# Disty0/sdnq

Hardware: AMD Instinct MI355X
Metric: quantized-matmul GOP/s (SDXL UNet int8 Linear step, bs=1) (higher is better)
Workload: dtype i8; 1 GPU; sdxl_int8: 741 quantized Linear layers of one denoising step, bs=1 (722 w8a8 GEMMs + 19 M=1 layers); parallelism=single GPU, launch=hipGraph replay, activations=bf16, distinct_activation_tensors=446, activation_quant_cache=True, requantized_weight_cache=True, fused_projections=False, linked_projection_groups=71, one_launch_linears=232, weights_dtype=int8, group_size=-1, use_quantized_matmul=True

## Files before the change

include/sdnq_hip.h:

```cpp
#ifndef SDNQ_HIP_H
#define SDNQ_HIP_H

#include <stddef.h>
#include <stdint.h>

#ifdef __cplusplus
extern "C" {
#endif

#define SDNQ_HIP_ABI_VERSION 1

typedef void* sdnq_stream_t;

typedef enum SdnqStatus {
    SDNQ_OK = 0,
    SDNQ_ERR_NULL = -1,
    SDNQ_ERR_DTYPE = -2,
    SDNQ_ERR_SHAPE = -3,
    SDNQ_ERR_ALIGN = -4,
    SDNQ_ERR_UNSUPPORTED = -5,
    SDNQ_ERR_ARCH = -6,
    SDNQ_ERR_LAUNCH = -7,
    SDNQ_ERR_WORKSPACE = -8
} SdnqStatus;
// ... 135 lines not shown
int sdnq_hip_lowrank_down(const void* x, int x_dtype, int64_t m, int64_t k, int64_t ldx, const void* svd_down,
                          int svd_dtype, int rank, void* t, sdnq_stream_t stream);

int sdnq_hip_scaled_mm_lowrank(int mm_dtype, const void* a, const void* b, const float* sa, const float* sb,
                               const void* bias, int bias_dtype, const void* t, const void* svd_up, int svd_dtype,
                               int rank, const int32_t* zp_rowsum, const float* zp, const float* a_zp,
                               const float* w_colsum_scaled, void* out, int out_dtype,
                               int64_t m, int64_t n, int64_t k, sdnq_stream_t stream);

int sdnq_hip_linear_float(const void* x, const void* wd, const void* bias, int dtype, void* out, int64_t m,
                          int64_t n, int64_t k, int64_t ldx, sdnq_stream_t stream);

int sdnq_hip_linear_skinny(const SdnqWeight* w, int hadamard_group, const void* x, const void* bias, int dtype, void* out,
                           int64_t m, int64_t ldx, sdnq_stream_t stream);

int sdnq_hip_quantize_weight(const void* src, int src_dtype, int64_t ld_src, const SdnqWeight* w, float qmin,
                             float qmax, sdnq_stream_t stream);

int sdnq_hip_quantize_codebook(const void* src, int src_dtype, int64_t ld_src, const SdnqWeight* w, int steps, sdnq_stream_t stream);

int sdnq_hip_prefetch(const void* ptr, int64_t bytes, int workgroups, sdnq_stream_t stream);
int sdnq_hip_prefetch_hint(const void* p0, int64_t b0, const void* p1, int64_t b1, const void* p2, int64_t b2, const void* p3, int64_t b3);

#define SDNQ_MAX_TP_RANKS 64
int sdnq_hip_unshard_columns(const void* gathered, void* out, int elem_bytes, int64_t m0, int64_t m_rows, int64_t m,
                             int64_t wmax, int world, const int64_t* starts, sdnq_stream_t stream);

#define SDNQ_MAX_PUSH_RANKS 16
#define SDNQ_SIGNAL_UNCACHED 1
#define SDNQ_SIGNAL_FINEGRAINED 2
#define SDNQ_SIGNAL_HOST_COHERENT 3
int sdnq_hip_signal_alloc(int64_t bytes, int kind, void** ptr, int* granted);
int sdnq_hip_signal_free(void* ptr, int kind);
int sdnq_hip_ipc_export(const void* ptr, void* handle64);
int sdnq_hip_ipc_import(const void* handle64, void** ptr);
int sdnq_hip_ipc_close(void* ptr);
int sdnq_hip_push_post(void* const* post, int world, int rank, uint64_t seq, uint64_t arena_offset, sdnq_stream_t stream);
int sdnq_hip_push_columns(const void* y, int elem_bytes, int64_t rows, int64_t w, int64_t ldy, void* const* arena, void* const* post,
                          void* const* done, int world, int rank, uint64_t seq, int64_t ldc, int64_t col0, int64_t row0, void* ticket,
                          void* status, int timeout_ms, sdnq_stream_t stream);

int sdnq_hip_im2col(const void* x, int dtype, int batch, int channels, int height, int width, int kh, int kw, int stride_h,
                    int stride_w, int pad_h, int pad_w, int dil_h, int dil_w, void* out, sdnq_stream_t stream);

int sdnq_hip_linear_w8a8(int mm_dtype, const void* x, int x_dtype, int64_t m, int64_t k, int64_t ldx, int hadamard_group,
                         void* xq, float* xs, const void* b, const float* sb, const void* bias, int bias_dtype, void* out,
                         int out_dtype, int64_t n, sdnq_stream_t stream);

int sdnq_hip_stream_capture_id(sdnq_stream_t stream, unsigned long long* id);

int sdnq_hip_linear_w8a8_fused(int mm_dtype, const void* x, int x_dtype, int64_t m, int64_t k, int64_t ldx, const void* b, const float* sb,
                               const void* bias, int bias_dtype, void* out, int out_dtype, int64_t n, sdnq_stream_t stream);
int sdnq_hip_linear_w8a8_fused_supported(int mm_dtype, int x_dtype, int out_dtype, int64_t m, int64_t n, int64_t k);

typedef struct SdnqLinearArgs {
    int32_t struct_size;
    int32_t mm_dtype;
    int32_t x_dtype;
    int32_t out_dtype;
    int32_t bias_dtype;
    int32_t svd_dtype;
    int32_t hadamard_group;
    int32_t svd_rank;
    int32_t asymmetric;
    int32_t x_prequantized;
    int64_t m, n, k, ldx;
    const void* x;
    void* out;
    const void* wq;
    const float* ws;
    const void* bias;
    const void* svd_down;
    const void* svd_up;
    const float* zp;
    const float* w_colsum_scaled;
    void* xq;
    float* xs;
    int32_t* rowsum;
    void* xrot;
    float* xzp;
    void* workspace;
    int64_t workspace_bytes;
} SdnqLinearArgs;
int sdnq_hip_linear(const SdnqLinearArgs* args, sdnq_stream_t stream);
int sdnq_hip_linear_workspace_bytes(const SdnqLinearArgs* args, int64_t* bytes);

int sdnq_hip_scaled_mm_nchw(int mm_dtype, const void* a, const void* b, const float* sa, const float* sb, const void* bias,
                            int bias_dtype, void* out, int out_dtype, int64_t m, int64_t n, int64_t k, int64_t hw,
                            sdnq_stream_t stream);

int sdnq_hip_scaled_mm_strided(int mm_dtype, const void* a, int64_t lda, const void* b, const float* sa, const float* sb,
                               const void* bias, int bias_dtype, void* out, int64_t ldc, int out_dtype, int64_t m, int64_t n,
                               int64_t k, int64_t hw, sdnq_stream_t stream);

int sdnq_hip_scaled_mm_lowrank_strided(int mm_dtype, const void* a, int64_t lda, const void* b, const float* sa, const float* sb,
                                       const void* bias, int bias_dtype, const int32_t* zp_rowsum, const float* zp, const float* a_zp,
                                       const float* w_colsum_scaled, int64_t zp_k, void* out, int64_t ldc, int out_dtype, int64_t m,
                                       int64_t n, int64_t k, sdnq_stream_t stream);

int sdnq_hip_linear_float_strided(const void* x, const void* wd, const void* bias, int dtype, void* out, int64_t m,
                                  int64_t n, int64_t k, int64_t ldx, int64_t ldc, sdnq_stream_t stream);

int sdnq_hip_im2col_rowquant(const void* x, int dtype, int batch, int channels, int height, int width, int kh, int kw,
                             int stride_h, int stride_w, int pad_h, int pad_w, int dil_h, int dil_w, int mm_dtype,
                             void* xq, float* xs, void* amax_ws, sdnq_stream_t stream);

// ... 127 lines not shown
```

sdnq_amd/csrc/gemm_aq.hip:

```cpp
#include "gemm_dev.h"
#include "quant8_dev.h"

namespace {

constexpr int BK = 128, NW = 8, NT = NW * 64;

struct AqParams {
    const float* sb;
    const void* bias;
    void* out;
    int64_t ldc;
    int bias_dtype;
    const uint8_t* pf_ptr[4];
    int pf_lines[4];
    unsigned long long* trace;
#ifdef SDNQ_AQ_LAB
    int lab;
#endif
};

typedef unsigned short us2 __attribute__((ext_vector_type(2)));

template <int MM> struct AqMma;
template <> struct AqMma<SDNQ_MM_I8> {
// ... 332 lines not shown
std::atomic<int> g_aq_geometry{-1};

constexpr int64_t AQ_TALL_MAX_K = 640;

struct AqPlan { int geometry, bm, bn, tiles_m, tiles_n, group_m, resident; int64_t prefetch_room; };
inline AqPlan aq_plan(int mm_dtype, int64_t m, int64_t n, int64_t k, int cus) {
    static const int geo_env = (int)env_int("SDNQ_HIP_FUSED_ROWQUANT_GEOMETRY", -1);
    static const int gm_env = (int)env_int("SDNQ_HIP_FUSED_ROWQUANT_GROUP_M", 8);
    static const int gm_tall_env = (int)env_int("SDNQ_HIP_FUSED_ROWQUANT_GROUP_M_TALL", 8);
    static const int tall = env_int("SDNQ_HIP_FUSED_ROWQUANT_TALL_GEOMETRY", 2) == 3 ? 3 : 2;
    struct Geo { int bm, bn, resident; };
    static constexpr Geo GEOS[4] = {{64, 128, 1}, {32, 256, 1}, {64, 128, 2}, {128, 128, 1}};
    const bool tall_ok = mm_dtype == SDNQ_MM_I8 && k <= AQ_TALL_MAX_K;
    auto tiles_of = [&](int g) { return ((m + GEOS[g].bm - 1) / GEOS[g].bm) * ((n + GEOS[g].bn - 1) / GEOS[g].bn); };
    int geo = g_aq_geometry.load(std::memory_order_relaxed);
    if (geo < 0) geo = geo_env;
    if (geo > 3 || (geo >= 2 && !tall_ok)) geo = -1;
    if (geo < 0) {
        if (mm_dtype == SDNQ_MM_I8 && k > 640 && (n % 256) == 0 && ((m + 31) / 32) * (n / 256) <= cus) geo = 1;
        else if (tall_ok && tiles_of(0) > cus && tiles_of(tall) <= (int64_t)GEOS[tall].resident * cus) geo = tall;
        else geo = 0;
    }
    AqPlan pl;
    pl.geometry = geo;
    pl.bm = GEOS[geo].bm;
    pl.bn = GEOS[geo].bn;
    pl.resident = GEOS[geo].resident;
    pl.tiles_m = (int)((m + pl.bm - 1) / pl.bm);
    pl.tiles_n = (int)((n + pl.bn - 1) / pl.bn);
    const int gm_e = geo >= 2 ? gm_tall_env : gm_env;
    const int gm = gm_e < 1 ? 1 : gm_e;
    pl.group_m = gm > pl.tiles_m ? pl.tiles_m : gm;
    pl.prefetch_room = (int64_t)pl.resident * cus - (int64_t)pl.tiles_m * pl.tiles_n;
    return pl;
}

template <int X_T, int MM, bool HAS_BIAS, int NJ, int NSB, int BM, int BN, int RESIDENT = 1>
int launch_aq(const void* x, const void* w, int64_t ldx, int64_t m, int64_t n, int64_t k, const AqPlan& pl, AqParams p, hipStream_t s) {
    constexpr int LDS_BYTES = NJ * BM * BK + NSB * BN * BK + (2 * BN + BM) * 4;
    static_assert(RESIDENT * LDS_BYTES <= 160 * 1024 && (RESIDENT + 1) * LDS_BYTES > 160 * 1024, "LDS budget: exactly RESIDENT workgroups per CU (aq_plan's prefetch room)");
    auto kern = linear_aq_kernel<X_T, MM, HAS_BIAS, NJ, NSB, BM, BN>;
    static std::atomic<uint64_t> attr_devices{0};
    if (LDS_BYTES > 64 * 1024 && !allow_dynamic_lds((const void*)kern, LDS_BYTES, attr_devices)) return SDNQ_ERR_LAUNCH;
    if (pl.bm != BM || pl.bn != BN || pl.resident != RESIDENT) return SDNQ_ERR_LAUNCH;
    const int tiles_m = pl.tiles_m, tiles_n = pl.tiles_n, group_m = pl.group_m;
    const int64_t tiles = (int64_t)tiles_m * tiles_n;
    p.trace = g_aq_trace.load(std::memory_order_relaxed);
#ifdef SDNQ_AQ_LAB
    p.lab = (int)env_int("SDNQ_HIP_AQ_LAB", 0);
#endif
    const int pf_wgs = sdnq_internal_take_prefetch(pl.prefetch_room, NT, p.pf_ptr, p.pf_lines);
    hipLaunchKernelGGL(kern, dim3((unsigned)(tiles + pf_wgs)), dim3(NT), LDS_BYTES, s, (const uint16_t*)x, (const uint8_t*)w, (int)ldx, (int)k, (int)m,
                       (int)n, (int)k, tiles_m, tiles_n, group_m, p);
    SDNQ_CHECK_LAUNCH();
    return SDNQ_OK;
}

}

extern "C" int sdnq_hip_linear_w8a8_fused_supported(int mm_dtype, int x_dtype, int out_dtype, int64_t m, int64_t n, int64_t k) {
    static const int64_t on = env_int("SDNQ_HIP_FUSED_ROWQUANT", 1), max_tn = env_int("SDNQ_HIP_FUSED_ROWQUANT_MAX_TILES_N", 12),
                         min_m = env_int("SDNQ_HIP_FUSED_ROWQUANT_MIN_M", 33), min_k = env_int("SDNQ_HIP_FUSED_ROWQUANT_MIN_K", 128),
                         max_k = env_int("SDNQ_HIP_FUSED_ROWQUANT_MAX_K", 1280);
    static const int64_t fp8_on = env_int("SDNQ_HIP_FUSED_ROWQUANT_FP8", 0);
    if (!on) return 0;
    if (mm_dtype != SDNQ_MM_I8 && !(mm_dtype == SDNQ_MM_FP8 && fp8_on)) return 0;
    if ((x_dtype != SDNQ_BF16 && x_dtype != SDNQ_F16) || out_dtype != x_dtype) return 0;
    if (m < min_m || n <= 0 || (n % 8) != 0 || k <= 0 || (k % 128) != 0 || k > 1280) return 0;
    const int64_t tiles_m = (m + 63) / 64, tiles_n = (n + 127) / 128;
    if (tiles_n > max_tn || k < min_k || k > max_k) return 0;
    if (tiles_m * tiles_n > (int64_t)cu_count() && aq_plan(mm_dtype, m, n, k, cu_count()).geometry < 2) return 0;
    return 1;
}

extern "C" int sdnq_hip_linear_w8a8_fused(int mm_dtype, const void* x, int x_dtype, int64_t m, int64_t k, int64_t ldx, const void* b,
                                          const float* sb, const void* bias, int bias_dtype, void* out, int out_dtype, int64_t n,
                                          sdnq_stream_t stream) {
    if (!x || !b || !sb || !out) return SDNQ_ERR_NULL;
    if (mm_dtype != SDNQ_MM_I8 && mm_dtype != SDNQ_MM_FP8) return SDNQ_ERR_DTYPE;
    if ((x_dtype != SDNQ_BF16 && x_dtype != SDNQ_F16) || out_dtype != x_dtype) return SDNQ_ERR_UNSUPPORTED;
    if (bias && (bias_dtype < 0 || bias_dtype > 2)) return SDNQ_ERR_DTYPE;
    if (m <= 0 || n <= 0 || k <= 0 || ldx < k || (n % 8) != 0) return SDNQ_ERR_SHAPE;
    if ((k % 128) != 0 || k > 1280) return SDNQ_ERR_UNSUPPORTED;
    if (m > 0x7fffffffll / 2 || n > 0x7fffffffll || ldx * 2 * 128 > 0x7fffffffll || k * 128 > 0x7fffffffll) return SDNQ_ERR_SHAPE;
    if (((uintptr_t)x % 16) || ((uintptr_t)b % 16) || ((uintptr_t)out % 16) || ((ldx * 2) % 16)) return SDNQ_ERR_ALIGN;
    AqParams p{};
    p.sb = sb; p.bias = bias; p.out = out; p.ldc = n; p.bias_dtype = bias_dtype;
    hipStream_t s = (hipStream_t)stream;
    const AqPlan pl = aq_plan(mm_dtype, m, n, k, cu_count());
#define AQ_L(XT, MMV, HB, NJV, ...) launch_aq<XT, MMV, HB, NJV, __VA_ARGS__>(x, b, ldx, m, n, k, pl, p, s)
#define AQ_G(XT, MMV, HB, NJV) (pl.geometry == 1 ? AQ_L(XT, MMV, HB, NJV, 3, 32, 256) : AQ_L(XT, MMV, HB, NJV, 4, 64, 128))
#define AQ_NJ(XT, MMV, HB) (k <= 640 ? AQ_G(XT, MMV, HB, 5) : AQ_G(XT, MMV, HB, 10))
#define AQ_B(XT, MMV) (bias ? AQ_NJ(XT, MMV, true) : AQ_NJ(XT, MMV, false))
#define AQ_X(MMV) (x_dtype == SDNQ_BF16 ? AQ_B(SDNQ_BF16, MMV) : AQ_B(SDNQ_F16, MMV))
#define AQ_TB(XT, ...) (bias ? AQ_L(XT, SDNQ_MM_I8, true, 5, __VA_ARGS__) : AQ_L(XT, SDNQ_MM_I8, false, 5, __VA_ARGS__))
#define AQ_T(...) (x_dtype == SDNQ_BF16 ? AQ_TB(SDNQ_BF16, __VA_ARGS__) : AQ_TB(SDNQ_F16, __VA_ARGS__))
    if (pl.geometry == 2) return AQ_T(2, 64, 128, 2);
    if (pl.geometry == 3) return AQ_T(3, 128, 128, 1);
    return mm_dtype == SDNQ_MM_I8 ? AQ_X(SDNQ_MM_I8) : AQ_X(SDNQ_MM_FP8);
#undef AQ_T
#undef AQ_TB
#undef AQ_X
#undef AQ_B
#undef AQ_NJ
#undef AQ_G
#undef AQ_L
}

void sdnq_internal_aq_trace(unsigned long long* device_buf) { g_aq_trace.store(device_buf, std::memory_order_relaxed); }

void sdnq_internal_aq_geometry(int geometry) { g_aq_geometry.store(geometry < 0 ? -1 : (geometry <= 3 ? geometry : 1), std::memory_order_relaxed); }

void sdnq_internal_aq_plan(int mm_dtype, long long m, long long n, long long k, int cus, long long* out) {
    const AqPlan pl = aq_plan(mm_dtype, m, n, k, cus);
    out[0] = pl.geometry; out[1] = pl.bm; out[2] = pl.bn; out[3] = pl.tiles_m; out[4] = pl.tiles_n; out[5] = pl.group_m; out[6] = pl.prefetch_room;
}
```

sdnq_amd/csrc/gemm_dev.h:

```cpp
#pragma once
#include <atomic>
#include <cstdlib>
#include <type_traits>

#include "sdnq_dev.h"

int sdnq_internal_take_prefetch(int64_t room, int threads, const uint8_t* pf_ptr[4], int pf_lines[4]);
int sdnq_float_gemm(const void* x, const void* w, const void* bias, int dtype, void* out, int64_t m, int64_t n, int64_t k,
                    int64_t ldx, hipStream_t s, void* const* outs = nullptr, int n_outs = 0, int64_t seg_n = 0, int64_t ldc = 0);
int sdnq_float_gemm_f32out(const void* x, const void* w, int dtype, float* out, int64_t m, int64_t n, int64_t k, int64_t ldx, int64_t ldc,
                           hipStream_t s);
bool sdnq_internal_ks_eligible(int64_t m, int64_t n, int64_t k, int64_t lda, int64_t ldb);
bool sdnq_internal_ks_preferred(int64_t m, int64_t n, int64_t k);
int sdnq_internal_scaled_mm_ks(const void* a, const void* b, const float* sa, const float* sb, const void* bias, int bias_dtype, void* out,
                               int out_dtype, int64_t m, int64_t n, int64_t k, int64_t lda, int64_t ldb, int64_t ldc, hipStream_t s);
void sdnq_internal_ks_trace(unsigned long long* device_buf);
void sdnq_internal_aq_trace(unsigned long long* device_buf);
void sdnq_internal_aq_geometry(int geometry);
void sdnq_internal_aq_plan(int mm_dtype, long long m, long long n, long long k, int cus, long long* out);

template <int N> __device__ __forceinline__ void wait_vmcnt() { asm volatile("s_waitcnt vmcnt(%0)" ::"n"(N) : "memory"); }

template <int N, int I = 0, typename F> __device__ __forceinline__ void static_for_up(F&& f) {
    if constexpr (I < N) {
        f(std::integral_constant<int, I>{});
        static_for_up<N, I + 1>(f);
    }
}

#define SDNQ_PHASE_STAMP(trace, slot)                                                                                                      \
    do {                                                                                                                                   \
        if ((trace) != nullptr && threadIdx.x == 0 && blockIdx.x < 1024) (trace)[blockIdx.x * 8 + (slot)] = __builtin_amdgcn_s_memtime(); \
    } while (0)

__device__ __forceinline__ int xcd_contiguous(int bid, int nwg) {
    const int q = nwg / 8, r = nwg % 8, xcd = bid % 8, j = bid / 8;
    return (xcd < r ? xcd * (q + 1) : r * (q + 1) + (xcd - r) * q) + j;
}

__device__ __forceinline__ void grouped_tile(int pos, int tiles_m, int tiles_n, int group_m, int& tile_m, int& tile_n) {
    const int per_group = group_m * tiles_n;
    const int gid = pos / per_group, first_m = gid * group_m;
    const int gsz = (tiles_m - first_m) < group_m ? (tiles_m - first_m) : group_m;
    const int in_g = pos - gid * per_group;
    tile_n = in_g / gsz;
    tile_m = first_m + in_g - tile_n * gsz;
}

#define SDNQ_PREFETCH_LINES(tid, wg, nt, nwgs, p)                                                                           \
    do {                                                                                                                    \
        const int t = (wg) * (nt) + (tid), stride = (nwgs) * (nt);                                                          \
        _Pragma("nounroll") for (int r = 0; r < 4; ++r) {                                                                   \
            const uint8_t* base = (p).pf_ptr[r];                                                                            \
            const int lines = (p).pf_lines[r];                                                                              \
            for (int i = t; i < lines; i += stride) {                                                                       \
                int v;                                                                                                      \
                asm volatile("global_load_dword %0, %1, off" : "=v"(v) : "v"(base + (int64_t)i * 128) : "memory");          \
            }                                                                                                               \
        }                                                                                                                   \
        asm volatile("s_waitcnt vmcnt(0)" ::: "memory");                                                                    \
    } while (0)

inline int64_t env_int(const char* name, int64_t dflt) {
    const char* e = getenv(name);
    return e ? atoll(e) : dflt;
}

inline int cu_count() {
    static std::atomic<int> cus[64];
    int dev = 0;
    if (hipGetDevice(&dev) != hipSuccess || dev < 0 || dev >= 64) return 256;
    int v = cus[dev].load(std::memory_order_relaxed);
// ... 18 lines not shown
```

sdnq_amd/linear.py:

```python
from __future__ import annotations

import functools
import os

import torch

from . import ops
from .common import dtype_dict

CACHE_WEIGHTS = os.environ.get("SDNQ_HIP_CACHE_WEIGHTS", "1").lower() not in {"0", "false", "no"}
PIPELINE_WEIGHTS = os.environ.get("SDNQ_HIP_PIPELINE_WEIGHTS", "0").lower() not in {"0", "false", "no"}
PREFETCH_WEIGHTS = os.environ.get("SDNQ_HIP_PREFETCH_WEIGHTS", "0").lower() not in {"0", "false", "no"}
PREFETCH_NEXT = os.environ.get("SDNQ_HIP_PREFETCH_NEXT", "1").lower() not in {"0", "false", "no"}
PREFETCH_NEXT_MAX_BYTES = int(os.environ.get("SDNQ_HIP_PREFETCH_NEXT_MAX_MB", "48")) << 20
FUSED_SKINNY = os.environ.get("SDNQ_HIP_FUSED_SKINNY", "1").lower() not in {"0", "false", "no"}
FUSED_DEQUANT_GEMM = os.environ.get("SDNQ_HIP_FUSED_DEQUANT_GEMM", "1").lower() not in {"0", "false", "no"}
FUSED_DEQUANT_GEMM_MAX_FLOP = float(os.environ.get("SDNQ_HIP_FUSED_DEQUANT_GEMM_MAX_FLOP", "4e10"))
FUSED_DEQUANT_GEMM_MAX_K = int(os.environ.get("SDNQ_HIP_FUSED_DEQUANT_GEMM_MAX_K", str(1 << 30)))
FUSED_ROWQUANT = os.environ.get("SDNQ_HIP_FUSED_ROWQUANT", "1").lower() not in {"0", "false", "no"}
FUSED_LUT4 = os.environ.get("SDNQ_HIP_FUSED_LUT4", "1").lower() not in {"0", "false", "no"}
CACHE_ACTIVATIONS = int(os.environ.get("SDNQ_HIP_CACHE_ACTIVATIONS", "12"))
_FP = ops._lib.fastpath()
FAST_PLANS = _FP is not None
_PLAN_NAMES = ("weight", "scale", "zero_point", "svd_up", "svd_down", "bias")
# ... 618 lines not shown
        members = []
        for m in self.mods:
            d = m.sdnq_dequantizer
            st = _state(m)
            bias = _attr(m, "bias")
            if (d.weights_dtype != "int8" or d.group_size > 0 or d.use_hadamard or d.kernel_positions != 1 or st.svd_up is not None
                    or d.in_features % 16 or (bias is not None and bias.dtype != input.dtype) or st.wd is not None):
                return False
            members.append((st.qw.keep[0].view(torch.int8).reshape(d.out_features, -1), st.qw.keep[1].reshape(-1), bias))
        try:
            self.gemm = ops.GemmGroup(members)
        except ops._lib.SdnqHipError:
            return False
        self.pf_tensors = tuple(w for (w, _, _) in members)
        return True

    def _claim(self, idx: int, input: torch.Tensor, key, stream):
        if self._c is not None:
            return self._c.claim(idx, input)
        last = self._last
        if last is None or last[0] is not input or last[1] != key or last[2] != stream or idx not in last[4]:
            return None
        y = last[3][idx].view(*input.shape[:-1], -1)
        last[4].discard(idx)
        if not last[4]:
            self._last = None
            self._wasted = 0
        return y

    def _begin_compute(self) -> bool:
        if (self._c.pending() if self._c is not None else (self._last is not None and self._last[4])):
            self.wasted += 1
            if self.wasted >= 2:
                fallback = self.fallback
                self.dissolve()
                if fallback:
                    from . import loader
                    for mods in fallback:
                        if all("_sdnq_group" not in m.__dict__ for m in mods):
                            loader.link_layers(mods)
                return False
        return True

    def forward(self, mod, idx: int, input: torch.Tensor, mm: int):
        key = None if _ts.no_reuse else tensor_key(input)
        if key is None:
            return None
        stream = ops._stream(input)
        y = self._claim(idx, input, key, stream)
        if y is not None:
            return y
        if not self._begin_compute() or not self._operands(mm):
            return None
        x2, xq, xs, _, _ = _rowquant_cached(input, input.shape[-1], mm, 0, False, False, None)
        if PREFETCH_NEXT:
            _pf_launch(self, self.pf_tensors)
        outs = ops.scaled_mm_grouped(mm, xq, xs, self.gemm, input.dtype)
        self.last = (input, key, stream, outs, set(range(len(self.mods))))
        if FAST_PLANS and self._c is not None and "_sdnq_plan" not in mod.__dict__:
            for i, m in enumerate(self.mods):
                if "_sdnq_plan" not in m.__dict__ and m.__dict__.get("_sdnq_group", (None,))[0] is self:
                    _install_plan(m, mm=mm, n=m.sdnq_dequantizer.out_features, k=m.sdnq_dequantizer.in_features, group=self._c,
                                  idx=m.__dict__["_sdnq_group"][1])
        return self._claim(idx, input, key, stream)

    def forward_float(self, mod, idx: int, input: torch.Tensor):
        key = tensor_key(input)
        if key is None:
            return None
        stream = ops._stream(input)
        y = self._claim(idx, input, key, stream)
        if y is not None:
            return y
        if not self._begin_compute():
            return None
        dq = mod.sdnq_dequantizer
        k, n = dq.in_features, dq.out_features
        x2 = input.reshape(-1, k)
        if x2.stride(-1) != 1 or (x2.stride(0) * x2.element_size()) % 16:
            x2 = x2.contiguous()
        g = len(self.mods)
        if FUSED_DEQUANT_GEMM and self._float_operands(input):
            if PREFETCH_NEXT:
                _pf_launch(self, self.pf_tensors)
            outs = ops.linear_w8a16_grouped(x2, self.gemm)
            self.last = (input, key, stream, outs, set(range(g)))
            return self._claim(idx, input, key, stream)
        wd = torch.empty((g * n, k), device=input.device, dtype=input.dtype)
        for i, m in enumerate(self.mods):
            d = m.sdnq_dequantizer
            ops.dequant(_state(m).qw, input.dtype, d.hadamard_group_size if d.use_hadamard else 0, out=wd[i * n:(i + 1) * n])
        biases = [_attr(m, "bias") for m in self.mods]
        bias = None if biases[0] is None else torch.cat(biases, dim=0)
        outs = ops.linear_float_multi(x2, wd, bias, g)
        self.last = (input, key, stream, outs, set(range(g)))
        return self._claim(idx, input, key, stream)


LINK_PROJECTIONS = os.environ.get("SDNQ_HIP_LINK_PROJECTIONS", "1").lower() not in {"0", "false", "no"}


def _quantized_matmul_forward(self, input: torch.Tensor, mm: int, small_batch_branch: bool = True, cache_input: bool = True) -> torch.Tensor:
    dq = self.sdnq_dequantizer
    st = _state(self)
    k, n = dq.in_features, dq.out_features
    m = input.numel() // input.shape[-1]
    if m == 0 or (small_batch_branch and m < 32):
        return _float_forward(self, input, st)
    if st.qw.scale_dtype != torch.float32:
        return _lp_matmul_forward(self, input, st, mm)
# ... 251 lines not shown
```

sdnq_amd/ops.py:

```python
from __future__ import annotations

import ctypes
import os
from dataclasses import dataclass

import torch

from . import _lib
from ._lib import BF16, F16, F32, MM_FP8, MM_I8, SdnqWeight, check
from .common import dtype_dict

_FLOAT_CODE = {torch.float32: F32, torch.bfloat16: BF16, torch.float16: F16}
_MM_TORCH = {MM_I8: torch.int8, MM_FP8: torch.float8_e4m3fn}


def float_code(dt: torch.dtype) -> int:
    try:
        return _FLOAT_CODE[dt]
    except KeyError:
        raise _lib.SdnqHipError(f"unsupported float dtype {dt}") from None


def mm_code(matmul_dtype: str) -> int:
    if matmul_dtype == "int8":
# ... 367 lines not shown
        scratch = torch.empty((xq_bytes + 4 * m + 512 + 255,), device=x2d.device, dtype=torch.uint8)
    else:
        scratch = _workspace(x2d.device, stream, xq_bytes + 4 * m + 512)
    base = (scratch.data_ptr() + 255) & ~255
    out = torch.empty((m, n), device=x2d.device, dtype=out_dtype)
    check(_lib.load().sdnq_hip_linear_w8a8(mm, x2d.data_ptr(), float_code(x2d.dtype), m, k, x2d.stride(0), hadamard_group, base,
                                           base + xq_bytes, b_phys.data_ptr(), sb.data_ptr(), _ptr(bias), 0 if bias is None else float_code(bias.dtype),
                                           out.data_ptr(), float_code(out_dtype), n, stream), "linear_w8a8")
    return out


def linear_w8a8_fused_supported(mm: int, x2d: torch.Tensor, n: int, out_dtype: torch.dtype) -> bool:
    if x2d.dtype not in (torch.bfloat16, torch.float16) or out_dtype != x2d.dtype or not x2d.is_cuda or x2d.stride(0) * 128 >= (1 << 31):
        return False
    key = (mm, x2d.dtype, x2d.shape[0], n, x2d.shape[1], x2d.device.index)
    r = _fused_ok.get(key)
    if r is None:
        with torch.cuda.device(x2d.device):
            r = bool(_lib.load().sdnq_hip_linear_w8a8_fused_supported(mm, float_code(x2d.dtype), float_code(out_dtype), x2d.shape[0], n, x2d.shape[1]))
        _fused_ok[key] = r
    return r


_fused_ok = {}
fused_calls = [0]


def fused_call_count() -> int:
    fp = _lib.fastpath()
    return fused_calls[0] + (fp.fused_calls() if fp is not None else 0)


def reset_fused_calls():
    fused_calls[0] = 0
    fp = _lib.fastpath()
    if fp is not None:
        fp.reset_counters()


def linear_w8a8_fused(mm: int, x2d: torch.Tensor, b_phys: torch.Tensor, sb: torch.Tensor, bias, out_dtype: torch.dtype) -> torch.Tensor:
    _require_cuda(x2d, b_phys, sb, bias)
    m, k = x2d.shape
    n = b_phys.shape[0]
    out = torch.empty((m, n), device=x2d.device, dtype=out_dtype)
    if bias is not None:
        bias = bias.contiguous()
    fused_calls[0] += 1
    check(_lib.load().sdnq_hip_linear_w8a8_fused(mm, x2d.data_ptr(), float_code(x2d.dtype), m, k, x2d.stride(0), b_phys.data_ptr(), sb.data_ptr(),
                                                 _ptr(bias), 0 if bias is None else float_code(bias.dtype), out.data_ptr(), float_code(out_dtype),
                                                 n, _stream(x2d)), "linear_w8a8_fused")
    return out


def scaled_mm_nchw(mm: int, a: torch.Tensor, b_phys: torch.Tensor, sa: torch.Tensor, sb: torch.Tensor, bias, out_dtype: torch.dtype,
                   batch: int, pixels: int) -> torch.Tensor:
    _require_cuda(a, b_phys, sa, sb, bias)
    m, k = a.shape
    n = b_phys.shape[0]
    assert m == batch * pixels
    out = torch.empty((batch, n, pixels), device=a.device, dtype=out_dtype)
    bias_dt = 0
    if bias is not None:
        bias = bias.contiguous()
        bias_dt = float_code(bias.dtype)
    check(_lib.load().sdnq_hip_scaled_mm_nchw(mm, a.data_ptr(), b_phys.data_ptr(), sa.data_ptr(), sb.data_ptr(), _ptr(bias), bias_dt,
                                              out.data_ptr(), float_code(out_dtype), m, n, k, pixels, _stream(a)), "scaled_mm_nchw")
    return out


def scaled_mm_into(mm: int, a: torch.Tensor, b_phys: torch.Tensor, sa: torch.Tensor, sb: torch.Tensor, bias, out: torch.Tensor,
                   chan0: int, pixels: int = 0) -> None:
    _require_cuda(a, b_phys, sa, sb, bias, out)
    m, k = a.shape
    n = b_phys.shape[0]
    assert a.stride(1) == 1 and b_phys.is_contiguous() and out.is_contiguous()
    c_total = out.shape[1]
    esz = out.element_size()
    dst = out.data_ptr() + (chan0 * pixels * esz if pixels else chan0 * esz)
    bias_dt = 0
    if bias is not None:
        bias = bias.contiguous()
        bias_dt = float_code(bias.dtype)
    check(_lib.load().sdnq_hip_scaled_mm_strided(mm, a.data_ptr(), a.stride(0), b_phys.data_ptr(), sa.data_ptr(), sb.data_ptr(), _ptr(bias),
                                                 bias_dt, dst, c_total, float_code(out.dtype), m, n, k, pixels, _stream(a)), "scaled_mm_strided")


def scaled_mm_zp_into(mm: int, a: torch.Tensor, b_phys: torch.Tensor, sa: torch.Tensor, sb: torch.Tensor, bias, rowsum, zp, a_zp, w_colsum_scaled,
                      zp_k: int, out: torch.Tensor, chan0: int) -> None:
    _require_cuda(a, b_phys, sa, sb, bias, rowsum, zp, a_zp, w_colsum_scaled, out)
    m, k = a.shape
    n = b_phys.shape[0]
    assert a.stride(1) == 1 and b_phys.is_contiguous() and out.is_contiguous() and out.dim() == 2
    bias_dt = 0
    if bias is not None:
        bias = bias.contiguous()
        bias_dt = float_code(bias.dtype)
    check(_lib.load().sdnq_hip_scaled_mm_lowrank_strided(mm, a.data_ptr(), a.stride(0), b_phys.data_ptr(), sa.data_ptr(), sb.data_ptr(), _ptr(bias),
                                                         bias_dt, _ptr(rowsum), _ptr(zp), _ptr(a_zp), _ptr(w_colsum_scaled), int(zp_k),
                                                         out.data_ptr() + chan0 * out.element_size(), out.shape[1], float_code(out.dtype), m, n, k,
                                                         _stream(a)), "scaled_mm_lowrank_strided")


def linear_float_into(x2d: torch.Tensor, w: torch.Tensor, bias, out: torch.Tensor, chan0: int) -> None:
    _require_cuda(x2d, w, bias, out)
    m, k = x2d.shape
    n = w.shape[0]
# ... 1015 lines not shown
```

Before: 628,400 GOP/s.

## Add fused row-quant grouped w8a8 kernel walking two N-tiles per workgroup

Adds a grouped variant of the fused activation-quantize + int8 GEMM kernel. It reads unit descriptors from a table so linked projection groups (for example QKV) can run in one launch without a separate row-quant kernel. Each workgroup quantizes its 32-row activation slab into LDS once and walks up to two 256-wide N tiles, reusing the quantized A across them. The weight-stream ring keeps running across the tile boundary. The Python grouped path uses it when supported and otherwise falls back to rowquant plus scaled_mm_grouped. This removes a kernel launch and the round trip of the quantized activation through memory, at the cost of a more complex kernel that only applies to K in 640..1280 with unit_n a multiple of 256.

```diff
diff --git a/include/sdnq_hip.h b/include/sdnq_hip.h
--- a/include/sdnq_hip.h
+++ b/include/sdnq_hip.h
@@ -211,6 +211,10 @@
 int sdnq_hip_linear_w8a8_fused(int mm_dtype, const void* x, int x_dtype, int64_t m, int64_t k, int64_t ldx, const void* b, const float* sb,
                                const void* bias, int bias_dtype, void* out, int out_dtype, int64_t n, sdnq_stream_t stream);
 int sdnq_hip_linear_w8a8_fused_supported(int mm_dtype, int x_dtype, int out_dtype, int64_t m, int64_t n, int64_t k);
+
+int sdnq_hip_linear_w8a8_fused_grouped(int mm_dtype, const void* x, int x_dtype, int64_t m, int64_t k, int64_t ldx, const SdnqGemmUnit* units,
+                                       int64_t n_units, int64_t unit_n, int bias_dtype, void* out, int out_dtype, sdnq_stream_t stream);
+int sdnq_hip_linear_w8a8_fused_grouped_supported(int mm_dtype, int x_dtype, int out_dtype, int64_t m, int64_t k, int64_t n_units, int64_t unit_n);
 
 typedef struct SdnqLinearArgs {
     int32_t struct_size;
diff --git a/sdnq_amd/csrc/gemm_aq.hip b/sdnq_amd/csrc/gemm_aq.hip
--- a/sdnq_amd/csrc/gemm_aq.hip
+++ b/sdnq_amd/csrc/gemm_aq.hip
@@ -408,6 +408,362 @@
     const int pf_wgs = sdnq_internal_take_prefetch(pl.prefetch_room, NT, p.pf_ptr, p.pf_lines);
     hipLaunchKernelGGL(kern, dim3((unsigned)(tiles + pf_wgs)), dim3(NT), LDS_BYTES, s, (const uint16_t*)x, (const uint8_t*)w, (int)ldx, (int)k, (int)m,
                        (int)n, (int)k, tiles_m, tiles_n, group_m, p);
+    SDNQ_CHECK_LAUNCH();
+    return SDNQ_OK;
+}
+
+constexpr int WALK_MAX = 2;
+
+struct AqWalkParams {
+    void* out;
+    int bias_dtype;
+    int ring_cold;
+    int pf_hosted;
+    const uint8_t* pf_ptr[4];
+    int pf_lines[4];
+    unsigned long long* trace;
+};
+
+#define SDNQ_WALK_STAMP(trace, slot)                                                                                                        \
+    do {                                                                                                                                   \
+        if ((trace) != nullptr && threadIdx.x == 0 && blockIdx.x < 512) (trace)[blockIdx.x * 16 + (slot)] = __builtin_amdgcn_s_memtime(); \
+    } while (0)
+
+template <int X_T, bool HAS_BIAS, int NJ>
+__global__ __launch_bounds__(NT) void linear_aq_walk_kernel(const uint16_t* __restrict__ x, const SdnqGemmUnit* __restrict__ units, int ldx, int M, int K,
+                                                            int tiles_m, int tiles_n, int wgs_n, int group_m, int walk, int unit_tiles,
+                                                            AqWalkParams p_) {
+    SDNQ_KERNARGS_NOW("s"(x), "s"(units), "s"(ldx), "s"(M), "s"(K), "s"(tiles_m), "s"(tiles_n), "s"(wgs_n), "s"(group_m), "s"(walk), "s"(unit_tiles), "s"(p_.out));
+    const AqWalkParams& p = p_;
+    constexpr int MM = SDNQ_MM_I8, BM = 32, BN = 256, NSB = 3, PPW = 4, DF = 2;
+    typedef AqMma<MM> MT;
+    constexpr int KS = BK / MT::KB, A_STAGE = BM * BK, B_STAGE = BN * BK, OUT_ROW = BN * 2 + 16;
+    static_assert(WALK_MAX == 2, "the tile after the first is the second: two weight descriptors, two output bases");
+    static_assert(NJ >= 2 * NSB, "the stream holds at least six stages: the drains under the quantization always refill");
+    extern __shared__ __attribute__((aligned(1024))) uint8_t lds[];
+    uint8_t* const ldsA = lds;
+    uint8_t* const ldsB = lds + NJ * A_STAGE;
+    float* const s_sb = (float*)(ldsB + NSB * B_STAGE);
+    float* const s_bias = s_sb + WALK_MAX * BN;
+    float* const s_xs = s_bias + WALK_MAX * BN;
+    uint8_t* const stg = (uint8_t*)(s_xs + BM);
+    uint64_t* const s_ob = (uint64_t*)(stg + BM * OUT_ROW);
+    int* const s_ldo = (int*)(s_ob + WALK_MAX);
+
+    const int tid = threadIdx.x, lane = tid & 63;
+    const int wave = __builtin_amdgcn_readfirstlane(tid >> 6);
+    const int nwg = tiles_m * wgs_n;
+    const int bid = blockIdx.x;
+    if (bid >= nwg) {
+        SDNQ_PREFETCH_LINES(tid, bid - nwg, NT, (int)gridDim.x - nwg, p);
+        return;
+    }
+    const unsigned long long t_entry = __builtin_amdgcn_s_memtime();
+    int tile_m, tile_w;
+    grouped_tile(xcd_contiguous(bid, nwg), tiles_m, wgs_n, group_m, tile_m, tile_w);
+    const int m0 = tile_m * BM, c0 = tile_w * walk;
+    const int nt = (tiles_n - c0) < walk ? (tiles_n - c0) : walk;
+    const int nk = K / BK;
+    const int m_rows = (M - m0) < BM ? (M - m0) : BM;
+
+    const auto rsX = SDNQ_MAKE_RSRC_N((const uint8_t*)x + (int64_t)m0 * ldx * 2, ((int64_t)(m_rows - 1) * ldx + K) * 2);
+    v4i xr[NJ];
+    const int qrow = wave * 4 + (lane >> 4);
+    {
+        const int rc = qrow < m_rows ? qrow : m_rows - 1;
+        const int vo = rc * ldx * 2 + (lane & 15) * 16;
+#pragma unroll
+        for (int j = 0; j < NJ; ++j) xr[j] = SDNQ_BUF_LOAD16(rsX, vo, j < nk ? j * 256 : 0x40000000);
+    }
+    const uint8_t* wb[WALK_MAX];
+    float ev_sb[WALK_MAX];
+    u32 ev_bias[WALK_MAX];
+#pragma unroll
+    for (int t = 0; t < WALK_MAX; ++t) {
+        const int c = c0 + (t < nt ? t : 0);
+        const int u = c / unit_tiles, d = (c - u * unit_tiles) * BN;
+        static_assert(sizeof(SdnqGemmUnit) == 40, "the table entry as five 64-bit words");
+        const auto* const uw = (const __attribute__((address_space(4))) uint64_t*)(uintptr_t)(units + u);
+        SdnqGemmUnit un;
+        un.b = (const void*)(uintptr_t)uw[0];
+        un.sb = (const float*)(uintptr_t)uw[1];
+        un.bias = (const void*)(uintptr_t)uw[2];
+        un.n_start = (int64_t)uw[3];
+        un.n_seg = (int32_t)(uint32_t)uw[4];
+        un.n_loc = (int32_t)(uint32_t)(uw[4] >> 32);
+        wb[t] = (const uint8_t*)un.b + (int64_t)d * K;
+        if (tid == 0) {
+            s_ob[t] = (uint64_t)(uintptr_t)p.out + (uint64_t)(((int64_t)M * un.n_start + un.n_loc + d) * 2);
+            s_ldo[t] = un.n_seg;
+        }
+        ev_sb[t] = 0.0f;
+        ev_bias[t] = 0;
+        if (tid < BN) {
+            ev_sb[t] = ((const __attribute__((address_space(1))) float*)(uintptr_t)un.sb)[d + tid];
+            if constexpr (HAS_BIAS) {
+                if (p.bias_dtype == SDNQ_F32) ev_bias[t] = ((const __attribute__((address_space(1))) u32*)(uintptr_t)un.bias)[d + tid];
+                else ev_bias[t] = ((const __attribute__((address_space(1))) uint16_t*)(uintptr_t)un.bias)[d + tid];
+            }
+        }
+    }
+    const auto rsB0 = SDNQ_MAKE_RSRC_N(wb[0], (int64_t)BN * K);
+    const auto rsB1 = SDNQ_MAKE_RSRC_N(wb[WALK_MAX - 1], (int64_t)BN * K);
+    int voB[PPW];
+#pragma unroll
+    for (int u = 0; u < PPW; ++u) {
+        const int r = (wave * PPW + u) * 8 + (lane >> 3);
+        voB[u] = r * K + (((lane & 7) ^ ((r >> 1) & 7)) << 4);
+    }
+    auto issueB = [&](bool second, int s, int slot) {
+        uint8_t* const dst = ldsB + slot * B_STAGE + wave * (PPW * 1024);
+        if (second) {
+#pragma unroll
+            for (int u = 0; u < PPW; ++u) SDNQ_DMA16(rsB1, dst + u * 1024, voB[u], s * BK);
+        } else {
+#pragma unroll
+            for (int u = 0; u < PPW; ++u) SDNQ_DMA16(rsB0, dst + u * 1024, voB[u], s * BK);
+        }
+    };
+#pragma unroll
+    for (int s = 0; s < NSB; ++s) issueB(false, s, s);
+    __builtin_amdgcn_sched_barrier(0);
+    SDNQ_KERNARGS_NOW("s"(p_.bias_dtype), "s"(p_.ring_cold), "s"(p_.pf_hosted), "s"(p_.trace));
+    if (p.trace != nullptr && tid == 0 && blockIdx.x < 512) p.trace[blockIdx.x * 16] = t_entry;
+    SDNQ_WALK_STAMP(p.trace, 1);
+
+    const bool cold = p.ring_cold != 0;
+    int slot = 0, tcur = 0;
+    int rem = (cold ? nk : nt * nk) - 1;
+    auto drainB = [&](int kt, typename MT::frag_t* dst) {
+        if (rem >= 2) wait_vmcnt<2 * PPW>();
+        else if (rem == 1) wait_vmcnt<PPW>();
+        else wait_vmcnt<0>();
+        static_for_up<KS>([&](auto ksc) { dst[decltype(ksc)::value] = MT::load(ldsB + slot * B_STAGE, wave * 32 + (lane & 31), decltype(ksc)::value, lane >> 5); });
+        asm volatile("s_waitcnt lgkmcnt(0)" ::: "memory");
+        if (rem >= NSB) {
+            const int s = kt + NSB;
+            if (s < nk) issueB(tcur != 0, s, slot);
+            else issueB(true, s - nk, slot);
+        }
+        slot = slot + 1 == NSB ? 0 : slot + 1;
+        --rem;
+    };
+
+    if (tid < BN) {
+#pragma unroll
+        for (int t = 0; t < WALK_MAX; ++t) {
+            s_sb[t * BN + tid] = ev_sb[t];
+            if constexpr (HAS_BIAS)
+                s_bias[t * BN + tid] = p.bias_dtype == SDNQ_F32 ? __uint_as_float(ev_bias[t])
+                                                                : (p.bias_dtype == SDNQ_BF16 ? __uint_as_float(ev_bias[t] << 16) : f16_bits_to_f32((uint16_t)ev_bias[t]));
+        }
+    }
+
+    constexpr float QMAX = 127.0f;
+    typename MT::frag_t fbr[DF][KS], fbs[KS];
+    {
+        wait_vmcnt<PPW * NSB>();
+        us2 mx = {0, 0};
+#pragma unroll
+        for (int j = 0; j < NJ; ++j)
+#pragma unroll
+            for (int d = 0; d < 4; ++d)
+                mx = __builtin_elementwise_max(mx, __builtin_bit_cast(us2, (u32)xr[j][d] & 0x7fff7fffu));
+        u32 m32 = __builtin_bit_cast(u32, mx);
+#pragma unroll
+        for (int s = 1; s <= 8; s <<= 1) {
+            const u32 o = (u32)lane_xor_i32((int)m32, s);
+            m32 = __builtin_bit_cast(u32, __builtin_elementwise_max(__builtin_bit_cast(us2, m32), __builtin_bit_cast(us2, o)));
+        }
+        u32 mb = (m32 & 0xffffu) > (m32 >> 16) ? (m32 & 0xffffu) : (m32 >> 16);
+        constexpr u32 INF_BITS = X_T == SDNQ_BF16 ? 0x7f80u : 0x7c00u;
+        if (__builtin_amdgcn_ballot_w64(mb > INF_BITS) != 0) {
+            u32 mn = 0;
+#pragma unroll
+            for (int j = 0; j < NJ; ++j)
+#pragma unroll
+                for (int d = 0; d < 4; ++d) {
+                    const u32 lo = (u32)xr[j][d] & 0x7fffu, hi = ((u32)xr[j][d] >> 16) & 0x7fffu;
+                    mn = lo > INF_BITS ? mn : (lo > mn ? lo : mn);
+                    mn = hi > INF_BITS ? mn : (hi > mn ? hi : mn);
+                }
+#pragma unroll
+            for (int s = 1; s <= 8; s <<= 1) {
+                const u32 o = (u32)lane_xor_i32((int)mn, s);
+                mn = o > mn ? o : mn;
+            }
+            mb = mn;
+        }
+        const float amax = X_T == SDNQ_BF16 ? __uint_as_float(mb << 16) : f16_bits_to_f32((uint16_t)mb);
+        const float scale = amax / QMAX;
+        RowDiv rd;
+        rd.set(scale);
+        if ((lane & 15) == 0) s_xs[qrow] = scale;
+        const int r = qrow;
+        uint8_t* dst = ldsA + r * 128 + ((lane & 1) << 3) + ((((lane & 15) >> 1) ^ ((r >> 1) & 7)) << 4);
+        const bool all_fast = __builtin_amdgcn_ballot_w64(!rd.fast) == 0;
+        if (all_fast) {
+#pragma unroll
+            for (int j = 0; j < NJ; ++j) {
+                float v[8];
+                const v4i t = xr[j];
+                Vec16<X_T>::unpack(make_uint4((u32)t[0], (u32)t[1], (u32)t[2], (u32)t[3]), v);
+                const uint2 q = quant8_fast<MM>(v, rd);
+                *(v2i*)(dst + j * A_STAGE) = (v2i){(int)q.x, (int)q.y};
+                if (j >= NJ - DF) drainB(j - (NJ - DF), fbr[j - (NJ - DF)]);
+            }
+        } else {
+#pragma unroll
+            for (int j = 0; j < NJ; ++j) {
+                float v[8];
+                const v4i t = xr[j];
+                Vec16<X_T>::unpack(make_uint4((u32)t[0], (u32)t[1], (u32)t[2], (u32)t[3]), v);
+                int isum = 0;
+                const uint2 q = quant8<MM>(v, rd, isum);
+                *(v2i*)(dst + j * A_STAGE) = (v2i){(int)q.x, (int)q.y};
+                if (j >= NJ - DF) drainB(j - (NJ - DF), fbr[j - (NJ - DF)]);
+            }
+        }
+    }
+    SDNQ_WALK_STAMP(p.trace, 2);
+
+    const int frow = lane & 31, fgrp = lane >> 5;
+    asm volatile("s_waitcnt lgkmcnt(0)" ::: "memory");
+    __builtin_amdgcn_s_barrier();
+    __builtin_amdgcn_sched_barrier(0);
+    typename MT::frag_t fa[2][KS];
+    auto read_a = [&](auto setc, auto ksc, int st) {
+        fa[decltype(setc)::value][decltype(ksc)::value] = MT::load(ldsA + (st < nk ? st : 0) * A_STAGE, frow, decltype(ksc)::value, fgrp);
+    };
+#pragma nounroll
+    for (int t = 0; t < nt; ++t) {
+        tcur = t;
+        if (cold && t > 0) {
+            rem = nk - 1;
+            slot = 0;
+#pragma unroll
+            for (int s = 0; s < NSB; ++s) issueB(true, s, s);
+        }
+        typename MT::acc_t acc;
+#pragma unroll
+        for (int e = 0; e < 16; ++e) acc[e] = 0;
+        static_for_up<KS>([&](auto ksc) { read_a(std::integral_constant<int, 0>{}, ksc, 0); });
+        static_for_up<NJ>([&](auto ktc) {
+            constexpr int kt = decltype(ktc)::value, sx = kt & 1;
+            if (kt < nk) {
+                if constexpr (kt < DF) {
+                    if (t == 0) {
+#pragma unroll
+                        for (int ks = 0; ks < KS; ++ks) fbs[ks] = fbr[kt][ks];
+                    } else {
+                        drainB(kt, fbs);
+                    }
+                } else {
+                    drainB(kt, fbs);
+                }
+                __builtin_amdgcn_sched_barrier(0);
+                static_for_up<KS>([&](auto ksc) {
+                    constexpr int ks = decltype(ksc)::value;
+                    MT::mma(acc, fbs[ks], fa[sx][ks]);
+                    __builtin_amdgcn_sched_barrier(0);
+                    if constexpr (kt + 1 < NJ) read_a(std::integral_constant<int, sx ^ 1>{}, ksc, kt + 1);
+                    __builtin_amdgcn_sched_barrier(0);
+                });
+            }
+        });
+        SDNQ_WALK_STAMP(p.trace, 3 + 4 * t);
+        if (t > 0) {
+            asm volatile("s_waitcnt lgkmcnt(0)" ::: "memory");
+            __builtin_amdgcn_s_barrier();
+        }
+        SDNQ_WALK_STAMP(p.trace, 4 + 4 * t);
+        {
+            const float sa = s_xs[frow];
+            const float* const t_sb = s_sb + t * BN;
+            const float* const t_bias = s_bias + t * BN;
+#pragma unroll
+            for (int q = 0; q < 4; ++q) {
+                const int nl0 = wave * 32 + 8 * q + 4 * fgrp;
+                float o[4];
+#pragma unroll
+                for (int e = 0; e < 4; ++e) {
+                    const float vv = MT::tof(acc, 4 * q + e) * sa;
+                    if constexpr (HAS_BIAS) o[e] = fmaf(vv, t_sb[nl0 + e], t_bias[nl0 + e]);
+                    else o[e] = vv * t_sb[nl0 + e];
+                }
+                *(v2i*)(stg + frow * OUT_ROW + nl0 * 2) = (v2i){(int)pack2<X_T>(o[0], o[1]), (int)pack2<X_T>(o[2], o[3])};
+            }
+        }
+        asm volatile("s_waitcnt lgkmcnt(0)" ::: "memory");
+        __builtin_amdgcn_s_barrier();
+        SDNQ_WALK_STAMP(p.trace, 5 + 4 * t);
+        {
+            const uint64_t o_t = s_ob[t];
+            const int64_t ld_t = s_ldo[t];
+            constexpr int PPR = BN * 2 / 16;
+#pragma unroll
+            for (int v = tid; v < BM * PPR; v += NT) {
+                const int r = v / PPR, c = v % PPR;
+                if (r >= m_rows) continue;
+                const v4i val = *(const v4i*)(stg + r * OUT_ROW + c * 16);
+                __builtin_nontemporal_store(val, (__attribute__((address_space(1))) v4i*)(uintptr_t)(o_t + (uint64_t)(((int64_t)(m0 + r) * ld_t + c * 8) * 2)));
+            }
+        }
+        SDNQ_WALK_STAMP(p.trace, 6 + 4 * t);
+    }
+    if (nt < walk && tile_m < p.pf_hosted) SDNQ_PREFETCH_LINES(tid, tile_m, NT, p.pf_hosted, p);
+}
+
+std::atomic<int> g_aq_walk{0};
+std::atomic<int> g_aq_group_route{-1};
+
+struct AqGroupPlan { int supported, tiles_m, tiles_n, walk, workgroups, singles, group_m; };
+inline AqGroupPlan aq_group_plan(int mm_dtype, int64_t m, int64_t unit_n, int64_t n_units, int64_t k, int cus) {
+    static const int walk_env = (int)env_int("SDNQ_HIP_FUSED_ROWQUANT_WALK", 0);
+    static const int gm_env = (int)env_int("SDNQ_HIP_FUSED_ROWQUANT_GROUP_M", 8);
+    AqGroupPlan pl{};
+    if (mm_dtype != SDNQ_MM_I8 || m < 33 || unit_n <= 0 || (unit_n % 256) != 0 || n_units <= 0 || (k % 128) != 0 || k <= 640 || k > 1280) return pl;
+    const int64_t tiles_m = (m + 31) / 32, tiles_n = n_units * (unit_n / 256);
+    if (tiles_m > 0x7fffffffll / 512 || tiles_n > 0x7fffffffll / 512) return pl;
+    int walk = g_aq_walk.load(std::memory_order_relaxed);
+    if (walk <= 0) walk = walk_env;
+    if (walk <= 0) {
+        for (walk = 1; walk < tiles_n && tiles_m * ((tiles_n + walk - 1) / walk) > cus; ++walk) {}
+    }
+    if (walk > tiles_n) walk = (int)tiles_n;
+    pl.tiles_m = (int)tiles_m;
+    pl.tiles_n = (int)tiles_n;
+    pl.walk = walk;
+    const int64_t wgs = tiles_m * ((tiles_n + walk - 1) / walk);
+    pl.workgroups = (int)(wgs < 0x7fffffffll ? wgs : 0x7fffffffll);
+    pl.singles = (tiles_n % walk) != 0 ? (int)tiles_m : 0;
+    const int gm = gm_env < 1 ? 1 : gm_env;
+    pl.group_m = gm > pl.tiles_m ? pl.tiles_m : gm;
+    pl.supported = walk <= WALK_MAX && wgs <= cus;
+    return pl;
+}
+
+template <int X_T, bool HAS_BIAS>
+int launch_aq_walk(const void* x, int64_t ldx, int64_t m, int64_t k, const SdnqGemmUnit* units, int64_t unit_n, const AqGroupPlan& pl, AqWalkParams p,
+                   hipStream_t s) {
+    constexpr int NJ = 10;
+    constexpr int LDS_BYTES = NJ * 32 * BK + 3 * 256 * BK + (2 * WALK_MAX * 256 + 32) * 4 + 32 * (256 * 2 + 16) + WALK_MAX * 16;
+    static_assert(LDS_BYTES <= 160 * 1024, "LDS budget: image + ring + per-channel vectors + output staging in one CU");
+    auto kern = linear_aq_walk_kernel<X_T, HAS_BIAS, NJ>;
+    static std::atomic<uint64_t> attr_devices{0};
+    if (!allow_dynamic_lds((const void*)kern, LDS_BYTES, attr_devices)) return SDNQ_ERR_LAUNCH;
+    static const int ring_cold = (int)env_int("SDNQ_HIP_FUSED_ROWQUANT_GROUPED_COLD_RING", 0);
+    static const int host_pf = (int)env_int("SDNQ_HIP_FUSED_ROWQUANT_GROUPED_PREFETCH", 1);
+    p.trace = g_aq_trace.load(std::memory_order_relaxed);
+    p.ring_cold = ring_cold;
+    const int64_t free_slots = (int64_t)cu_count() - pl.workgroups;
+    int pf_wgs = 0;
+    p.pf_hosted = 0;
+    if (free_slots > 0) pf_wgs = sdnq_internal_take_prefetch(free_slots, NT, p.pf_ptr, p.pf_lines);
+    else p.pf_hosted = sdnq_internal_take_prefetch(host_pf ? pl.singles : 0, NT, p.pf_ptr, p.pf_lines);
+    const int wgs_n = pl.workgroups / pl.tiles_m;
+    hipLaunchKernelGGL(kern, dim3((unsigned)(pl.workgroups + pf_wgs)), dim3(NT), LDS_BYTES, s, (const uint16_t*)x, units, (int)ldx, (int)m, (int)k, pl.tiles_m,
+                       pl.tiles_n, wgs_n, pl.group_m, pl.walk, (int)(unit_n / 256), p);
     SDNQ_CHECK_LAUNCH();
     return SDNQ_OK;
 }
@@ -463,6 +819,46 @@
 #undef AQ_L
 }
 
+extern "C" int sdnq_hip_linear_w8a8_fused_grouped_supported(int mm_dtype, int x_dtype, int out_dtype, int64_t m, int64_t k, int64_t n_units,
+                                                            int64_t unit_n) {
+    static const int64_t on = env_int("SDNQ_HIP_FUSED_ROWQUANT", 1), grouped_on = env_int("SDNQ_HIP_FUSED_ROWQUANT_GROUPED", 1);
+    const int forced = g_aq_group_route.load(std::memory_order_relaxed);
+    if (!on || !(forced < 0 ? grouped_on != 0 : forced != 0)) return 0;
+    if ((x_dtype != SDNQ_BF16 && x_dtype != SDNQ_F16) || out_dtype != x_dtype) return 0;
+    return aq_group_plan(mm_dtype, m, unit_n, n_units, k, cu_count()).supported;
+}
+
+extern "C" int sdnq_hip_linear_w8a8_fused_grouped(int mm_dtype, const void* x, int x_dtype, int64_t m, int64_t k, int64_t ldx,
+                                                  const SdnqGemmUnit* units, int64_t n_units, int64_t unit_n, int bias_dtype, void* out,
+                                                  int out_dtype, sdnq_stream_t stream) {
+    if (!x || !units || !out) return SDNQ_ERR_NULL;
+    if (mm_dtype != SDNQ_MM_I8 && mm_dtype != SDNQ_MM_FP8) return SDNQ_ERR_DTYPE;
+    if ((x_dtype != SDNQ_BF16 && x_dtype != SDNQ_F16) || out_dtype != x_dtype) return SDNQ_ERR_UNSUPPORTED;
+    if (bias_dtype > 2) return SDNQ_ERR_DTYPE;
+    if (m <= 0 || n_units <= 0 || unit_n <= 0 || (unit_n % 64) != 0 || k <= 0 || ldx < k) return SDNQ_ERR_SHAPE;
+    if ((k % 128) != 0 || k > 1280) return SDNQ_ERR_UNSUPPORTED;
+    if (m > 0x7fffffffll / 2 || n_units * unit_n > 0x7fffffffll || ldx * 2 * 128 > 0x7fffffffll || k * 256 > 0x7fffffffll) return SDNQ_ERR_SHAPE;
+    if (((uintptr_t)x % 16) || ((uintptr_t)units % 8) || ((uintptr_t)out % 16) || ((ldx * 2) % 16)) return SDNQ_ERR_ALIGN;
+    const AqGroupPlan pl = aq_group_plan(mm_dtype, m, unit_n, n_units, k, cu_count());
+    if (!pl.supported) return SDNQ_ERR_UNSUPPORTED;
+    AqWalkParams p{};
+    p.out = out; p.bias_dtype = bias_dtype < 0 ? 0 : bias_dtype;
+    hipStream_t s = (hipStream_t)stream;
+#define AQ_W(XT) (bias_dtype >= 0 ? launch_aq_walk<XT, true>(x, ldx, m, k, units, unit_n, pl, p, s) : launch_aq_walk<XT, false>(x, ldx, m, k, units, unit_n, pl, p, s))
+    return x_dtype == SDNQ_BF16 ? AQ_W(SDNQ_BF16) : AQ_W(SDNQ_F16);
+#undef AQ_W
+}
+
+void sdnq_internal_aq_group_force(int walk, int route) {
+    g_aq_walk.store(walk < 0 ? 0 : walk, std::memory_order_relaxed);
+    g_aq_group_route.store(route < 0 ? -1 : (route != 0), std::memory_order_relaxed);
+}
+
+void sdnq_internal_aq_group_plan(int mm_dtype, long long m, long long unit_n, long long n_units, long long k, int cus, long long* out) {
+    const AqGroupPlan pl = aq_group_plan(mm_dtype, m, unit_n, n_units, k, cus);
+    out[0] = pl.supported; out[1] = pl.tiles_m; out[2] = pl.tiles_n; out[3] = pl.walk; out[4] = pl.workgroups; out[5] = pl.singles; out[6] = pl.group_m;
+}
+
 void sdnq_internal_aq_trace(unsigned long long* device_buf) { g_aq_trace.store(device_buf, std::memory_order_relaxed); }
 
 void sdnq_internal_aq_geometry(int geometry) { g_aq_geometry.store(geometry < 0 ? -1 : (geometry <= 3 ? geometry : 1), std::memory_order_relaxed); }
diff --git a/sdnq_amd/csrc/gemm_dev.h b/sdnq_amd/csrc/gemm_dev.h
--- a/sdnq_amd/csrc/gemm_dev.h
+++ b/sdnq_amd/csrc/gemm_dev.h
@@ -18,6 +18,8 @@
 void sdnq_internal_aq_trace(unsigned long long* device_buf);
 void sdnq_internal_aq_geometry(int geometry);
 void sdnq_internal_aq_plan(int mm_dtype, long long m, long long n, long long k, int cus, long long* out);
+void sdnq_internal_aq_group_force(int walk, int route);
+void sdnq_internal_aq_group_plan(int mm_dtype, long long m, long long unit_n, long long n_units, long long k, int cus, long long* out);
 
 template <int N> __device__ __forceinline__ void wait_vmcnt() { asm volatile("s_waitcnt vmcnt(%0)" ::"n"(N) : "memory"); }
 
diff --git a/sdnq_amd/linear.py b/sdnq_amd/linear.py
--- a/sdnq_amd/linear.py
+++ b/sdnq_amd/linear.py
@@ -694,10 +694,21 @@
             return y
         if not self._begin_compute() or not self._operands(mm):
             return None
-        x2, xq, xs, _, _ = _rowquant_cached(input, input.shape[-1], mm, 0, False, False, None)
-        if PREFETCH_NEXT:
-            _pf_launch(self, self.pf_tensors)
-        outs = ops.scaled_mm_grouped(mm, xq, xs, self.gemm, input.dtype)
+        outs, hinted = None, False
+        if FUSED_ROWQUANT:
+            x2 = input if input.dim() == 2 else input.reshape(-1, input.shape[-1])
+            if x2.stride(-1) != 1 or (x2.stride(0) * x2.element_size()) % 16:
+                x2 = x2.contiguous()
+            if ops.linear_w8a8_fused_grouped_supported(mm, x2, self.gemm, input.dtype):
+                if PREFETCH_NEXT:
+                    _pf_launch(self, self.pf_tensors)
+                    hinted = True
+                outs = ops.linear_w8a8_fused_grouped(mm, x2, self.gemm, input.dtype)
+        if outs is None:
+            x2, xq, xs, _, _ = _rowquant_cached(input, input.shape[-1], mm, 0, False, False, None)
+            if PREFETCH_NEXT and not hinted:
+                _pf_launch(self, self.pf_tensors)
+            outs = ops.scaled_mm_grouped(mm, xq, xs, self.gemm, input.dtype)
         self.last = (input, key, stream, outs, set(range(len(self.mods))))
         if FAST_PLANS and self._c is not None and "_sdnq_plan" not in mod.__dict__:
             for i, m in enumerate(self.mods):
diff --git a/sdnq_amd/ops.py b/sdnq_amd/ops.py
--- a/sdnq_amd/ops.py
+++ b/sdnq_amd/ops.py
@@ -443,6 +443,43 @@
     return out
 
 
+_fused_group_ok = {}
+
+
+def linear_w8a8_fused_grouped_supported(mm: int, x2d: torch.Tensor, group: GemmGroup, out_dtype: torch.dtype) -> bool:
+    if x2d.dtype not in (torch.bfloat16, torch.float16) or out_dtype != x2d.dtype or not x2d.is_cuda or x2d.stride(0) * 128 >= (1 << 31):
+        return False
+    if x2d.shape[1] != group.k or x2d.device != group.device:
+        return False
+    key = (mm, x2d.dtype, x2d.shape[0], group.k, group.n_units, group.unit_n, x2d.device.index)
+    r = _fused_group_ok.get(key)
+    if r is None:
+        with torch.cuda.device(x2d.device):
+            r = bool(_lib.load().sdnq_hip_linear_w8a8_fused_grouped_supported(mm, float_code(x2d.dtype), float_code(out_dtype), x2d.shape[0],
+                                                                              group.k, group.n_units, group.unit_n))
+        _fused_group_ok[key] = r
+    return r
+
+
+def linear_w8a8_fused_grouped(mm: int, x2d: torch.Tensor, group: GemmGroup, out_dtype: torch.dtype):
+    _require_cuda(x2d)
+    m, k = x2d.shape
+    if k != group.k:
+        raise _lib.SdnqHipError(f"grouped matmul: activation has K={k}, the group K={group.k}")
+    out = torch.empty((m * group.n_total,), device=x2d.device, dtype=out_dtype)
+    st = _lib.load().sdnq_hip_linear_w8a8_fused_grouped(mm, x2d.data_ptr(), float_code(x2d.dtype), m, k, x2d.stride(0), group.table.data_ptr(),
+                                                        group.n_units, group.unit_n, group.bias_dtype, out.data_ptr(), float_code(out_dtype),
+                                                        _stream(x2d))
+    if st == _lib.ERR_UNSUPPORTED:
+        return None
+    check(st, "linear_w8a8_fused_grouped")
+    outs, start = [], 0
+    for n in group.widths:
+        outs.append(out[m * start:m * (start + n)].view(m, n))
+        start += n
+    return outs
+
+
 def scaled_mm_nchw(mm: int, a: torch.Tensor, b_phys: torch.Tensor, sa: torch.Tensor, sb: torch.Tensor, bias, out_dtype: torch.dtype,
                    batch: int, pixels: int) -> torch.Tensor:
     _require_cuda(a, b_phys, sa, sb, bias)
```

After: 626,100 GOP/s. No clear change (-0.4%).
